# ssydasheng/GPflow-Slim

Hardware: AMD Instinct MI355X
Metric: GPR log-marginal-likelihood evals/sec + predict_f latency, fp64, N=32768 D=8 (higher is better)
Workload: dtype f64; 1 GPU; RBF(ARD) GPR log-marginal-likelihood, N=32768 D=8 R=1 fp64, X resident in HBM; n=32768, d=8, n_new=1024, parallelism=1 GPU (fused single-GPU path)

## Files before the change

gpflow-slim_amd/csrc/gps_handle.hip:

```cpp
#include "gps_ops.hpp"

extern "C" int gps_create(int device_id, gps_handle_t* out) {
  if (!out) return GPS_ERR_ARG;
  *out = nullptr;
  int count = 0;
  if (hipGetDeviceCount(&count) != hipSuccess || count <= 0) return GPS_ERR_HIP;
  if (device_id < 0 || device_id >= count) return GPS_ERR_ARG;
  gps_handle_t h = new gps_handle_s();
  h->device = device_id;
  if (hipSetDevice(device_id) != hipSuccess || hipGetDeviceProperties(&h->prop, device_id) != hipSuccess) {
    delete h;
    return GPS_ERR_HIP;
  }
  if (hipStreamCreateWithFlags(&h->stream, hipStreamNonBlocking) != hipSuccess) { delete h; return GPS_ERR_HIP; }
  for (int i = 0; i < 8; ++i) {
    if (hipEventCreate(&h->ev[i]) != hipSuccess) { delete h; return GPS_ERR_HIP; }
  }
  if (const char* v = getenv("GPS_GEMM_PAIR")) h->gemm_pair = atoi(v);
  if (const char* la = getenv("GPS_LOOKAHEAD")) h->potrf_lookahead = atoi(la);
  if (h->dInfo.ensure(64) != hipSuccess || h->dScal.ensure(4096) != hipSuccess) { delete h; return GPS_ERR_HIP; }
  *out = h;
  return GPS_OK;
}

// ... 187 lines not shown
  GPS_HIP(h, hipMemcpyAsync(h->dTmp2.p, B, bb, hipMemcpyHostToDevice, h->stream));
  GPS_HIP(h, hipMemcpyAsync(h->dTmp3.p, C, cb, hipMemcpyHostToDevice, h->stream));
  GemmBatch bt; bt.batch = batch; bt.a_rs = m; bt.b_rs = n; bt.c_rs = m;
  int rc = gps_launch_gemm_nt_ex(h, op, 0, tri, m, n, k, h->dTmp.d(), k, h->dTmp2.d(), k, h->dTmp3.d(), n, &bt);
  if (rc) return rc;
  GPS_HIP(h, hipMemcpyAsync(C, h->dTmp3.p, cb, hipMemcpyDeviceToHost, h->stream));
  GPS_HIP(h, hipStreamSynchronize(h->stream));
  return GPS_OK;
}

extern "C" int gps_diag_gemm_timeline(gps_handle_t h, int op, int lower, int64_t m, int64_t n, int64_t k, int reps,
                                      long long* stamps_out, int64_t cap_blocks, int64_t* nblocks, double* ms_per_launch) {
  if (!h || !stamps_out || cap_blocks <= 0 || reps <= 0) return GPS_ERR_ARG;
  GPS_HIP(h, hipSetDevice(h->device));
  return gps_run_gemm_timeline(h, op, lower, m, n, k, reps, stamps_out, cap_blocks, nblocks, ms_per_launch);
}

extern "C" int gps_diag_potrf_base_stamps(gps_handle_t h, int factor, double* us_out7) {
  if (!h || !us_out7) return GPS_ERR_ARG;
  GPS_HIP(h, hipSetDevice(h->device));
  const size_t bb = (size_t)GPS_TILE * GPS_TILE * 8;
  GPS_HIP(h, h->dTmp.ensure(4 * bb + 2048));
  std::vector<double> A((size_t)GPS_TILE * GPS_TILE, 0.0);
  for (int i = 0; i < GPS_TILE; ++i) for (int j = 0; j <= i; ++j) A[(size_t)i * GPS_TILE + j] = (i == j) ? 2.0 + 0.01 * i : 0.3 / (1.0 + i - j);
  double* dA = h->dTmp.d();
  long long* dS = (long long*)(dA + 3 * GPS_TILE * GPS_TILE);
  long long hs[96] = {0};
  const bool per_wave = getenv("GPS_PB_WAVE_STAMPS") != nullptr;
  for (int rep = 0; rep < 3; ++rep) {
    GPS_HIP(h, hipMemsetAsync(dS, 0, 96 * sizeof(long long), h->stream));
    if (per_wave) { const long long one = 1; GPS_HIP(h, hipMemcpyAsync(dS + 31, &one, sizeof(one), hipMemcpyHostToDevice, h->stream)); }
    GPS_HIP(h, hipMemcpyAsync(dA, A.data(), bb, hipMemcpyHostToDevice, h->stream));
    int rc = gps_launch_fill_info(h, (int*)h->dInfo.p, INT_MAX);
    if (rc) return rc;
    rc = gps_launch_potrf_base(h, dA, GPS_TILE, dA + GPS_TILE * GPS_TILE, getenv("GPS_PB_NO_T") ? nullptr : dA + 2 * GPS_TILE * GPS_TILE,
                               (int*)h->dInfo.p, 0, factor, dS);
    if (rc) return rc;
    GPS_HIP(h, hipMemcpyAsync(hs, dS, sizeof(hs), hipMemcpyDeviceToHost, h->stream));
    GPS_HIP(h, hipStreamSynchronize(h->stream));
  }
  for (int q = 0; q < 7; ++q) us_out7[q] = (double)(hs[q] - hs[0]) * 0.01;
  us_out7[0] = (double)(hs[8 + 2] - hs[8 + 1]) / ((double)(hs[2] - hs[1]) * 0.01);
  if (factor) {
    fprintf(stderr, "potrf_base phases (us): A (panel | update + inverse in its shadow) %.2f  B (next block column) %.2f\n", hs[16] * 0.01, hs[17] * 0.01);
    for (int g = 0; g < 8 && per_wave; ++g) {
      fprintf(stderr, "  step %d: per-wave end of phase A (us):", g);
      for (int w = 0; w < 8; ++w) fprintf(stderr, " %.2f", hs[32 + 8 * g + w] * 0.01);
      fprintf(stderr, "\n");
    }
  }
  return GPS_OK;
}

static int diag_trsm512_impl(gps_handle_t h, int64_t m, int backward, int panel, int reps, double* us_per_solve,
                             double* maxdiff_out, long long* stamps_out, int64_t cap_blocks) {
  if (!h || m <= 0 || m % GPS_TILE || reps <= 0 || !us_per_solve) return GPS_ERR_ARG;
  GPS_HIP(h, hipSetDevice(h->device));
  const i64 T = GPS_TILE, n = 4 * T;
  std::vector<double> L((size_t)n * n, 0.0), B((size_t)T * n);
  unsigned long long st = 88172645463325252ull;
  auto rnd = [&]() { st ^= st << 13; st ^= st >> 7; st ^= st << 17; return (double)(st >> 11) / 9007199254740992.0 - 0.5; };
  for (i64 i = 0; i < n; ++i) for (i64 j = 0; j <= i; ++j) L[i * n + j] = (i == j) ? 2.0 + 0.5 * (rnd() + 0.5) : 0.1 * rnd();
  for (auto& v : B) v = rnd();
  GPS_HIP(h, h->dTmp.ensure((size_t)2 * n * n * 8));
  GPS_HIP(h, h->dTmp3.ensure((size_t)8 * T * T * 8));
  GPS_HIP(h, h->dB.ensure((size_t)m * n * 8 * 3));
  double* dL = h->dTmp.d(); double* dU = dL + n * n; double* dInv = h->dTmp3.d(); double* dInvT = dInv + 4 * T * T;
  double* dBm = h->dB.d(); double* dB0 = dBm + m * n; double* dB1 = dB0 + m * n;
  GPS_HIP(h, hipMemcpyAsync(dL, L.data(), (size_t)n * n * 8, hipMemcpyHostToDevice, h->stream));
  for (i64 q = 0; q < m / T; ++q) GPS_HIP(h, hipMemcpyAsync(dB0 + q * T * n, B.data(), (size_t)T * n * 8, hipMemcpyHostToDevice, h->stream));
  int rc = gps_launch_transpose(h, dL, n, n, n, dU, n);
  if (rc) return rc;
  rc = gps_launch_fill_info(h, (int*)h->dInfo.p, INT_MAX);
  if (rc) return rc;
  HipOps ops{h, dInv, dInvT, (int*)h->dInfo.p};
  ops.factor = 0;
  for (i64 b = 0; b < 4 && !rc; ++b) rc = ops.potrf_base(dL + b * T * n + b * T, n, b, b * T);
  if (rc) return rc;
  Blocked<HipOps> bl(ops);
  const bool saved_ref = h->refine_now; const int saved_panel = h->trsm_panel;
  h->refine_now = false;
  auto solve = [&](double* X) -> int { return backward ? bl.trsm_rn_rec(dU, n, n, 0, X, n, m) : bl.trsm_rec(dL, n, n, 0, X, n, m); };
  hipEvent_t e0, e1;
  GPS_HIP(h, hipEventCreate(&e0)); GPS_HIP(h, hipEventCreate(&e1));
  float ms = 0.f;
  h->trsm_panel = panel;
  for (int pass = 0; pass < 2 && !rc; ++pass) {
    GPS_HIP(h, hipEventRecord(e0, h->stream));
    for (int it = 0; it < reps && !rc; ++it) {
      if (it == 0 || it == reps - 1) GPS_HIP(h, hipMemcpyAsync(dBm, dB0, (size_t)m * n * 8, hipMemcpyDeviceToDevice, h->stream));
      rc = solve(dBm);
    }
    GPS_HIP(h, hipEventRecord(e1, h->stream));
    GPS_HIP(h, hipStreamSynchronize(h->stream));
    GPS_HIP(h, hipEventElapsedTime(&ms, e0, e1));
  }
  if (!rc && stamps_out) {
    const i64 nb = std::min<i64>(m / 32, cap_blocks);
    GPS_HIP(h, h->dGemvWs.ensure((size_t)(m / 32) * 32 * sizeof(long long)));
    GPS_HIP(h, hipMemsetAsync(h->dGemvWs.p, 0, (size_t)(m / 32) * 32 * sizeof(long long), h->stream));
    GPS_HIP(h, hipMemcpyAsync(dBm, dB0, (size_t)m * n * 8, hipMemcpyDeviceToDevice, h->stream));
    h->tp_stamps = (long long*)h->dGemvWs.p;
    rc = solve(dBm);
    h->tp_stamps = nullptr;
    GPS_HIP(h, hipMemcpyAsync(stamps_out, h->dGemvWs.p, (size_t)nb * 32 * sizeof(long long), hipMemcpyDeviceToHost, h->stream));
    GPS_HIP(h, hipStreamSynchronize(h->stream));
// ... 102 lines not shown
```

gpflow-slim_amd/csrc/potrf_base.hip:

```cpp
#include "gps_common.hpp"

#define PB 128
#define PS 129
#define NT 512
typedef double v4d __attribute__((ext_vector_type(4)));
typedef double v2d_ __attribute__((ext_vector_type(2)));

#ifndef GPS_PB_WT
#define GPS_PB_WT 0
#endif
__device__ __forceinline__ void pb_store16(double* p, double2 v) {
#if GPS_PB_WT
  v2d_ w; w.x = v.x; w.y = v.y;
  asm volatile("global_store_dwordx4 %0, %1, off sc1\n\ts_nop 1" :: "v"(p), "v"(w) : "memory");
#else
  *reinterpret_cast<double2*>(p) = v;
#endif
}
typedef __attribute__((address_space(3))) int lds_int;

__device__ __forceinline__ void load_image(double* a, const double* __restrict__ A, i64 lda, int tid) {
  double2 v[16];
#pragma unroll
  for (int u = 0; u < 16; ++u) {
    const int idx = u * NT + tid;
    const int i = idx >> 6, j = (idx & 63) * 2;
    v[u] = *reinterpret_cast<const double2*>(A + (i64)i * lda + j);
  }
#pragma unroll
  for (int u = 0; u < 16; ++u) {
    const int idx = u * NT + tid;
    const int i = idx >> 6, j = (idx & 63) * 2;
    a[i * PS + j] = v[u].x;
    a[i * PS + j + 1] = v[u].y;
  }
}

__device__ __forceinline__ double x_elem(const double* a, const double* dinv, int r, int c) {
  double off = a[(r > c) ? (c * PS + r) : 0];
  double dia = dinv[r & (PB - 1)];
  asm volatile("" : "+v"(off), "+v"(dia));
  return (r > c) ? off : ((r == c) ? dia : 0.0);
}

#define PB_FMAC_DPP(d, a, b, k) asm volatile("v_fmac_f64_dpp %0, %1, -%2 row_newbcast:%3 row_mask:0xf bank_mask:0xf" : "+v"(d) : "v"(a), "v"(b), "n"(k))
#define PB_MOV_DPP(d, a, k) asm volatile("v_mov_b64_dpp %0, %1 row_newbcast:%2 row_mask:0xf bank_mask:0xf" : "=v"(d) : "v"(a), "n"(k))
#define PB_SCALE2(a, b, y) asm volatile("v_mul_f64 %0, %0, %2\n\tv_mul_f64 %1, %1, %2\n\ts_nop 1" : "+v"(a), "+v"(b) : "v"(y))
#define PB_UPD2(J, K) do { PB_FMAC_DPP(r[K], r[J], r[J], K); PB_FMAC_DPP(x[K], r[J], x[J], K); } while (0)

template <int J>
__device__ __forceinline__ void pb_pivot(double (&r)[16], double (&x)[16], double& p, double& y, double& sd, double& dd, int& bad) {
#define PB_FENCE() __builtin_amdgcn_sched_barrier(0)
  const double lj = sd * y;
  PB_SCALE2(r[J], x[J], y);
  PB_FENCE();
  const double pn = __builtin_fma(-lj, lj, dd);
  if constexpr (J + 1 < 16) PB_UPD2(J, J + 1);
// ... 111 lines not shown
  for (int rg = 0; rg < 4; ++rg) acc[rg] = pc[4 * rg * PS];
  for (int p = 0; p < np; ++p) {
    const int q = (p + 1 < np) ? p + 1 : p;
    double an[4], bn[4];
#pragma unroll
    for (int s4 = 0; s4 < 4; ++s4) { an[s4] = pa[16 * q + 4 * s4]; bn[s4] = pb[16 * q + 4 * s4]; }
    __builtin_amdgcn_sched_barrier(0);
#pragma unroll
    for (int s4 = 0; s4 < 4; ++s4) acc = __builtin_amdgcn_mfma_f64_16x16x4f64(-av[s4], bv[s4], acc, 0, 0, 0);
#pragma unroll
    for (int s4 = 0; s4 < 4; ++s4) { av[s4] = an[s4]; bv[s4] = bn[s4]; }
  }
#pragma unroll
  for (int rg = 0; rg < 4; ++rg) pc[4 * rg * PS] = acc[rg];
}

__device__ __forceinline__ int q_pull(int* counter, int lane) {
  int t = 0;
  if (lane == 0) t = atomicAdd(counter, 1);
  return __builtin_amdgcn_readfirstlane(t);
}

template <int NR>
__device__ __forceinline__ void store_L_rows(const double* a, double* __restrict__ A, i64 lda, int i0, int lane) {
  const int j = 2 * lane;
  char* base = reinterpret_cast<char*>(A + (i64)i0 * lda) + 16 * lane;
  const unsigned step = (unsigned)lda * 8u;
  double2 v[NR];
#pragma unroll
  for (int u = 0; u < NR; ++u) { v[u].x = a[(i0 + u) * PS + j]; v[u].y = a[(i0 + u) * PS + j + 1]; }
#pragma unroll
  for (int u = 0; u < NR; ++u) {
    const int i = i0 + u;
    v[u].x = (j <= i) ? v[u].x : 0.0;
    v[u].y = (j + 1 <= i) ? v[u].y : 0.0;
    pb_store16(reinterpret_cast<double*>(base + (size_t)(u * step)), v[u]);
  }
}
template <int NR>
__device__ __forceinline__ void store_inv_rows(const double* a, const double* dinv, double* __restrict__ Linv, int i0, int lane) {
  const int c = 2 * lane;
  double2 v[NR];
  double d[NR];
#pragma unroll
  for (int u = 0; u < NR; ++u) { v[u].x = a[c * PS + i0 + u]; v[u].y = a[(c + 1) * PS + i0 + u]; d[u] = dinv[i0 + u]; }
#pragma unroll
  for (int u = 0; u < NR; ++u) {
    const int i = i0 + u;
    v[u].x = (i > c) ? v[u].x : ((i == c) ? d[u] : 0.0);
    v[u].y = (i > c + 1) ? v[u].y : ((i == c + 1) ? d[u] : 0.0);
    pb_store16(Linv + i * PB + c, v[u]);
  }
}
__device__ __forceinline__ void inv_diag16(double* a, const double* dinv, int c) {
  const int rem = 15 - (c & 15);
  double x[16];
  x[0] = dinv[c];
#pragma unroll
  for (int d = 1; d < 16; ++d) {
    if (d <= rem) {
      const int i = c + d;
      double s = a[i * PS + c] * x[0];
#pragma unroll
      for (int t = 1; t < d; ++t) s += a[i * PS + c + t] * x[t];
      x[d] = -s * dinv[i];
    }
  }
#pragma unroll
  for (int d = 1; d < 16; ++d)
    if (d <= rem) a[c * PS + c + d] = x[d];
}

__device__ __forceinline__ void inv_row_tile(double* a, const double* dinv, int gp, int c, int fr, int fk) {
  v4d t0 = (v4d){0.0, 0.0, 0.0, 0.0}, t1 = (v4d){0.0, 0.0, 0.0, 0.0};
  const double* la = a + (16 * gp + fr) * PS + fk;
  const double* xb = a + (16 * c + fr) * PS + fk;
  double av[4], bv[4];
#pragma unroll
  for (int s = 0; s < 4; ++s) {
    av[s] = la[16 * c + 4 * s];
    bv[s] = x_elem(a, dinv, 16 * c + 4 * s + fk, 16 * c + fr);
  }
  for (int kb = c + 1; kb < gp; ++kb) {
    double an[4], bn[4];
#pragma unroll
    for (int s = 0; s < 4; ++s) { an[s] = la[16 * kb + 4 * s]; bn[s] = xb[16 * kb + 4 * s]; }
    t0 = __builtin_amdgcn_mfma_f64_16x16x4f64(av[0], bv[0], t0, 0, 0, 0);
    t1 = __builtin_amdgcn_mfma_f64_16x16x4f64(av[1], bv[1], t1, 0, 0, 0);
    t0 = __builtin_amdgcn_mfma_f64_16x16x4f64(av[2], bv[2], t0, 0, 0, 0);
    t1 = __builtin_amdgcn_mfma_f64_16x16x4f64(av[3], bv[3], t1, 0, 0, 0);
#pragma unroll
    for (int s = 0; s < 4; ++s) { av[s] = an[s]; bv[s] = bn[s]; }
  }
  double xv[4];
#pragma unroll
  for (int s = 0; s < 4; ++s) xv[s] = x_elem(a, dinv, 16 * gp + fr, 16 * gp + 4 * s + fk);
  t0 = __builtin_amdgcn_mfma_f64_16x16x4f64(av[0], bv[0], t0, 0, 0, 0);
  t1 = __builtin_amdgcn_mfma_f64_16x16x4f64(av[1], bv[1], t1, 0, 0, 0);
  t0 = __builtin_amdgcn_mfma_f64_16x16x4f64(av[2], bv[2], t0, 0, 0, 0);
  t1 = __builtin_amdgcn_mfma_f64_16x16x4f64(av[3], bv[3], t1, 0, 0, 0);
  t0 += t1;
  v4d z = (v4d){0.0, 0.0, 0.0, 0.0};
#pragma unroll
  for (int s = 0; s < 4; ++s) z = __builtin_amdgcn_mfma_f64_16x16x4f64(xv[s], t0[s], z, 0, 0, 0);
#pragma unroll
  for (int rg = 0; rg < 4; ++rg) a[(16 * c + fr) * PS + 16 * gp + fk + 4 * rg] = -z[rg];
}

__device__ __forceinline__ void potrf_base_body(char* smem_raw, double* __restrict__ A, i64 lda, double* __restrict__ Linv,
                                                double* __restrict__ LinvT, int* __restrict__ info, int row0, int factor,
                                                long long* __restrict__ stamps) {
#define STAMP(q) do { if (stamps && threadIdx.x == 0) { stamps[q] = (long long)wall_clock64(); stamps[8 + q] = (long long)clock64(); } } while (0)
  STAMP(0);
  double* a = reinterpret_cast<double*>(smem_raw);
  double* dinv = a + PB * PS;

  const int tid = threadIdx.x;
  const int lane = tid & 63, wave = __builtin_amdgcn_readfirstlane(tid >> 6);
  const int fr = lane & 15, fk = lane >> 4;

  int* q_mfma = reinterpret_cast<int*>(dinv + PB + 192);
  int* q_store = q_mfma + 9;
  lds_int* pflag = (lds_int*)(q_store + 8);
  __syncthreads();
  if (tid < 18) q_mfma[tid] = 0;
  load_image(a, A, lda, tid);
  __syncthreads();
  STAMP(1);

  int tail_row0 = 0;
  int flag_sum = 0;
  if (factor) {
    long long t_a = 0, t_b = 0, t0 = 0;
    for (int g = 0; g < 8; ++g) {
      const int o = 16 * g;
      const int nrows = PB - o - 16;
      const int npanel = nrows > 96 ? 3 : (nrows > 32 ? 2 : 1);
      if (stamps && (tid == 0 || (lane == 0 && stamps[31]))) t0 = (long long)wall_clock64();
      if (wave < npanel) {
        flag_sum += npanel - 1;
        panel_step_dpp(a, info, row0, o, lane, wave, npanel, pflag, flag_sum);
      } else if (g >= 1) {
        {
          const int n_inv = g - 1, n_ll = (g <= 6) ? 7 - g : 0, n_items = n_inv + n_ll;
          for (int it = q_pull(q_mfma + g, lane); it < n_items; it = q_pull(q_mfma + g, lane)) {
            if (n_inv > 0 && it == 0) inv_row_tile(a, dinv, g - 1, 0, fr, fk);
            else if (it - (n_inv > 0 ? 1 : 0) < n_ll) lookleft_tile(a, g + 1 + it - (n_inv > 0 ? 1 : 0), g + 1, g, fr, fk);
            else inv_row_tile(a, dinv, g - 1, it - n_ll, fr, fk);
          }
        }
        for (int it = q_pull(q_store + g, lane); it < 4; it = q_pull(q_store + g, lane))
          store_L_rows<4>(a, A, lda, 16 * (g - 1) + 4 * it, lane);
      }
      if (stamps && lane == 0 && stamps[31]) stamps[32 + 8 * g + wave] = (long long)wall_clock64() - t0;
      __syncthreads();
      if (stamps && tid == 0) { const long long t1 = (long long)wall_clock64(); t_a += t1 - t0; t0 = t1; }
      if (wave == 0) { }
      else {
        const int I = g + wave;
        if (I < 8) update_tile(a, I, g + 1, o, fr, fk);
      }
      __syncthreads();
      if (stamps && tid == 0) t_b += (long long)wall_clock64() - t0;
    }
    if (stamps && tid == 0) { stamps[16] = t_a; stamps[17] = t_b; stamps[18] = 0; }
    STAMP(2);
    STAMP(3);
    STAMP(4);
    if (wave < 7) inv_row_tile(a, dinv, 7, wave, fr, fk);
    {
      for (int it = q_pull(q_mfma + 8, lane); it < 4 + 28; it = q_pull(q_mfma + 8, lane)) {
        if (it < 4) store_L_rows<4>(a, A, lda, 112 + 4 * it, lane);
        else store_inv_rows<4>(a, dinv, Linv, 4 * (it - 4), lane);
      }
    }
    tail_row0 = 112;
    __syncthreads();
  } else {
    if (tid < PB) dinv[tid] = 1.0 / a[tid * PS + tid];
    __syncthreads();
    STAMP(2); STAMP(3);
    if (tid < PB) inv_diag16(a, dinv, tid);
    __syncthreads();
    STAMP(4);
    for (int gp = 1; gp < 8; ++gp) {
      if (wave < gp) inv_row_tile(a, dinv, gp, wave, fr, fk);
      __syncthreads();
    }
  }

  STAMP(5);
  {
    const int i0 = 0, w2 = PB / 2;
    for (int idx = tail_row0 * 64 + tid; idx < PB * PB / 2; idx += NT) {
      const int i = idx >> 6, c = (idx & 63) * 2;
      double2 v;
      v.x = x_elem(a, dinv, i, c);
      v.y = x_elem(a, dinv, i, c + 1);
      pb_store16(Linv + i * PB + c, v);
    }
    if (LinvT) {
      for (int idx = tid; idx < PB * w2; idx += NT) {
        const int c = idx / w2, i = i0 + 2 * (idx - c * w2);
        double2 v;
        v.x = x_elem(a, dinv, i, c);
        v.y = x_elem(a, dinv, i + 1, c);
        pb_store16(LinvT + c * PB + i, v);
      }
    }
  }
  __syncthreads();
  STAMP(6);
#undef STAMP
}


#define PB_LDS_BYTES ((PB * PS + PB + 192 + 10) * 8)

#ifndef GPS_PB_DEVICE_ONLY
__global__ __launch_bounds__(NT) __attribute__((amdgpu_waves_per_eu(2, 2))) void potrf_base_kernel(double* __restrict__ A, i64 lda,
                                                        double* __restrict__ Linv,
                                                        double* __restrict__ LinvT,
                                                        int* __restrict__ info, int row0,
                                                        int factor, long long* __restrict__ stamps) {
  extern __shared__ __attribute__((aligned(16))) char smem_raw[];
  potrf_base_body(smem_raw, A, lda, Linv, LinvT, info, row0, factor, stamps);
}

int gps_launch_potrf_base(gps_handle_t h, double* A, i64 lda, double* Linv_blk,
                          double* LinvT_blk, int* d_info, i64 row0, int factor, long long* d_stamps) {
  const size_t lds = (size_t)PB_LDS_BYTES;
  int rc0 = gps_dyn_lds(h, reinterpret_cast<const void*>(&potrf_base_kernel), (int)lds);
  if (rc0) return rc0;
  LaunchScope ls(h, KC_POTRF_BASE, 2.0 * PB * PB * PB / 3.0, 3.0 * PB * PB * 8.0);
  hipLaunchKernelGGL(potrf_base_kernel, dim3(1), dim3(NT), lds, h->stream, A, lda, Linv_blk,
                     LinvT_blk, d_info, (int)row0, factor, d_stamps);
  GPS_HIP(h, hipGetLastError());
  return GPS_OK;
}
#endif
```

gpflow-slim_amd/gpflowSlim/_backend.py:

```python
import ctypes
import os
import threading

import numpy as np

GPS_MAX_DIMS = 32
GPS_MAX_NODES = 64
GPS_MAX_STACK = 4

K_RBF, K_MATERN12, K_MATERN32, K_MATERN52, K_PERIODIC, K_WHITE, K_CONSTANT, K_EXPONENTIAL = 1, 2, 3, 4, 5, 6, 7, 8
K_SQDIST, K_EUCLID = 9, 10
K_ADD, K_MUL = 16, 17
K_NKN_LINROW, K_NKN_PRODUCT, K_NKN_ACT = 32, 33, 34

_c_double_p = ctypes.POINTER(ctypes.c_double)
_c_int_p = ctypes.POINTER(ctypes.c_int)
_i64 = ctypes.c_int64


class KernNode(ctypes.Structure):
    _fields_ = [("op", ctypes.c_int32),
                ("n_dims", ctypes.c_int32),
                ("active_dims", ctypes.c_int32 * GPS_MAX_DIMS),
                ("variance", ctypes.c_double),
# ... 93 lines not shown
                      _c_double_p, _c_double_p, _c_double_p, _c_int_p],
    "gps_fitc": [ctypes.c_void_p, ctypes.POINTER(KernNode), ctypes.c_int, _c_double_p, _i64, _c_double_p, _i64, _i64,
                 ctypes.c_double, ctypes.c_double, _c_double_p, _i64, _c_double_p, _i64, ctypes.c_int, _c_double_p,
                 _c_double_p, _c_double_p, _c_int_p],
    "gps_sparse_last_terms": [ctypes.c_void_p, _c_double_p],
    "gps_profile_enable": [ctypes.c_void_p, ctypes.c_int],
    "gps_profile_reset": [ctypes.c_void_p],
    "gps_profile_get": [ctypes.c_void_p, ctypes.c_char_p, ctypes.POINTER(_i64), _c_double_p, _c_double_p,
                        _c_double_p],
    "gps_last_stage_ms": [ctypes.c_void_p, _c_double_p],
    "gps_set_option": [ctypes.c_void_p, ctypes.c_char_p, ctypes.c_double],
    "gps_set_stream": [ctypes.c_void_p, ctypes.c_void_p, ctypes.c_int],
    "gps_dist_begin": [ctypes.c_void_p, ctypes.POINTER(KernNode), ctypes.c_int, ctypes.c_double, _c_double_p, _i64,
                       ctypes.c_int, ctypes.c_int, _i64, ctypes.POINTER(_i64), ctypes.POINTER(_i64)],
    "gps_dist_msg_doubles": [ctypes.c_void_p, _i64, ctypes.POINTER(_i64)],
    "gps_dist_set_comm": [ctypes.c_void_p, ctypes.c_void_p, ctypes.c_void_p],
    "gps_dist_set_comm_bufs": [ctypes.c_void_p, ctypes.POINTER(ctypes.c_void_p), ctypes.c_int],
    "gps_dist_comm_bufs_needed": [ctypes.c_void_p, _c_int_p],
    "gps_device_bytes": [ctypes.c_void_p, ctypes.POINTER(_i64)],
    "gps_dist_solve_begin": [ctypes.c_void_p, ctypes.POINTER(KernNode), ctypes.c_int, _c_double_p, _i64],
    "gps_dist_solve_pack": [ctypes.c_void_p, _i64, ctypes.c_int],
    "gps_dist_grad_begin": [ctypes.c_void_p],
    "gps_dist_grad_fwd_apply": [ctypes.c_void_p, _i64, ctypes.c_int],
    "gps_dist_grad_bwd_apply": [ctypes.c_void_p, _i64, ctypes.c_int],
    "gps_dist_grad_local": [ctypes.c_void_p, ctypes.POINTER(KernNode), ctypes.c_int, _c_double_p, ctypes.c_int, _c_int_p, _c_double_p],
    "gps_dist_grad_fold": [ctypes.c_void_p, ctypes.POINTER(KernNode), ctypes.c_int, _c_double_p, ctypes.c_int, _i64, _c_double_p,
                           ctypes.c_int, _c_int_p, _c_double_p],
    "gps_dist_lml_grad": [ctypes.c_void_p, ctypes.POINTER(KernNode), ctypes.c_int, ctypes.c_double, _c_double_p, _i64, _i64,
                          ctypes.c_int, ctypes.c_int, _c_double_p, _c_double_p, ctypes.c_int, _c_int_p, _c_double_p, _c_double_p,
                          _c_int_p],
    "gps_dist_solve_apply": [ctypes.c_void_p, _i64, ctypes.c_int],
    "gps_dist_solve_finish": [ctypes.c_void_p, ctypes.POINTER(KernNode), ctypes.c_int, _c_double_p, _c_double_p],
    "gps_dist_lml": [ctypes.c_void_p, ctypes.POINTER(KernNode), ctypes.c_int, ctypes.c_double, _c_double_p, _i64, _i64, ctypes.c_int,
                     ctypes.c_int, _c_double_p, _c_int_p],
    "gps_dist_predict": [ctypes.c_void_p, ctypes.POINTER(KernNode), ctypes.c_int, _c_double_p, _i64, ctypes.c_int, _c_double_p, _c_double_p],
    "gps_dist_panel_factor": [ctypes.c_void_p, _i64, ctypes.c_int],
    "gps_dist_unpack": [ctypes.c_void_p, _i64, ctypes.c_int],
    "gps_dist_update": [ctypes.c_void_p, _i64, _i64, _i64, ctypes.c_int],
    "gps_dist_set_bulk_stream": [ctypes.c_void_p, ctypes.c_void_p],
    "gps_dist_finish": [ctypes.c_void_p, _c_double_p, _c_int_p],
    "gps_comm_load": [ctypes.c_char_p],
    "gps_comm_version": [_c_int_p],
    "gps_comm_unique_id": [ctypes.c_void_p, ctypes.c_int],
    "gps_comm_init": [ctypes.c_void_p, ctypes.c_int, ctypes.c_int, ctypes.c_void_p, ctypes.c_int],
    "gps_comm_destroy": [ctypes.c_void_p],
    "gps_comm_abort": [ctypes.c_void_p],
    "gps_comm_exchange": [ctypes.c_void_p, ctypes.c_void_p, _i64, ctypes.c_int, ctypes.c_int, ctypes.c_int],
    "gps_comm_wait": [ctypes.c_void_p, ctypes.c_int],
    "gps_comm_allreduce": [ctypes.c_void_p, ctypes.c_void_p, _i64],
    "gps_comm_install_allreduce": [ctypes.c_void_p, ctypes.c_void_p, _i64],
    "gps_set_allreduce": [ctypes.c_void_p, ctypes.c_void_p, ctypes.c_void_p, ctypes.c_void_p, _i64],
    "gps_allreduce_doubles": [_i64, _i64, ctypes.POINTER(_i64)],
    "gps_diag_potrf_base_stamps": [ctypes.c_void_p, ctypes.c_int, _c_double_p],
    "gps_diag_mfma_f64": [ctypes.c_void_p, ctypes.c_int, _c_double_p, _c_int_p],
    "gps_diag_gemm_nt": [ctypes.c_void_p, ctypes.c_int, ctypes.c_int, _i64, _i64, _i64, _c_double_p, _c_double_p,
                         _c_double_p],
    "gps_diag_gemm_nt_batched": [ctypes.c_void_p, ctypes.c_int, ctypes.c_int, _i64, _i64, _i64, _i64, _c_double_p, _c_double_p,
                                 _c_double_p],
    "gps_diag_trsm512": [ctypes.c_void_p, _i64, ctypes.c_int, ctypes.c_int, ctypes.c_int, _c_double_p, _c_double_p],
    "gps_diag_trsm512_stamps": [ctypes.c_void_p, _i64, ctypes.c_int, ctypes.c_int, _c_double_p, ctypes.POINTER(ctypes.c_longlong), _i64],
    "gps_diag_trsm_leaf": [ctypes.c_void_p, _i64, ctypes.c_int, ctypes.c_int, ctypes.c_int, _c_double_p, _c_double_p],
    "gps_diag_set_cu_mask": [ctypes.c_void_p, ctypes.POINTER(ctypes.c_uint32), ctypes.c_int],
    "gps_diag_gemm_timeline": [ctypes.c_void_p, ctypes.c_int, ctypes.c_int, _i64, _i64, _i64, ctypes.c_int,
                               ctypes.POINTER(ctypes.c_longlong), _i64, ctypes.POINTER(ctypes.c_int64), _c_double_p],
}
EXPORTED_SYMBOLS = sorted(list(_SIGNATURES) + ["gps_last_error", "gps_comm_load_error"])
ALLREDUCE_FN = ctypes.CFUNCTYPE(ctypes.c_int, ctypes.c_void_p, ctypes.c_void_p, _i64)

_lib = None
_lib_lock = threading.Lock()


def _share_hip_runtime_with_torch():
    if os.environ.get("GPFLOWSLIM_NO_TORCH_RUNTIME"):
        return
    try:
        import importlib.util
        spec = importlib.util.find_spec("torch")
        if spec is None or not spec.submodule_search_locations:
            return
        cand = os.path.join(list(spec.submodule_search_locations)[0], "lib", "libamdhip64.so")
        if os.path.exists(cand):
            ctypes.CDLL(cand, mode=ctypes.RTLD_GLOBAL)
    except Exception:
        pass


def load_library():
    global _lib
    with _lib_lock:
        if _lib is not None:
            return _lib
        path = lib_path()
        if not os.path.exists(path):
            raise RuntimeError(
                "gpflowSlim (MI355X): HIP library not found at %s -- build it with "
                "`make -C gpflow-slim_amd/csrc` (or __graft_entry__.build()). There is no CPU fallback." % path)
        _share_hip_runtime_with_torch()
        lib = ctypes.CDLL(path)
        for name, argtypes in _SIGNATURES.items():
            try:
                fn = getattr(lib, name)
            except AttributeError:
                if os.environ.get("GPFLOWSLIM_HIP_LIB"):
                    continue
                raise
# ... 278 lines not shown
            raise NotPositiveDefiniteError(
                "Cholesky decomposition was not successful: leading minor of order %d is not positive definite" % info.value)
        return lml.value

    def dist_predict(self, prog, Xnew, r, exchange_mode):
        Xnew = _f64(Xnew)
        n_new = Xnew.shape[0]
        mean = np.empty((n_new, max(r, 1)))
        var = np.empty(n_new)
        self._check(self._lib.gps_dist_predict(self._h, prog, len(prog), _ptr(Xnew) if n_new else None, n_new, int(exchange_mode),
                                               _ptr(mean) if n_new else None, _ptr(var) if n_new else None), "gps_dist_predict")
        return mean[:, :r], var

    def dist_panel_factor(self, j, buf):
        self._check(self._lib.gps_dist_panel_factor(self._h, int(j), int(buf)), "gps_dist_panel_factor")

    def dist_unpack(self, j, buf):
        self._check(self._lib.gps_dist_unpack(self._h, int(j), int(buf)), "gps_dist_unpack")

    def dist_update(self, j, c_lo, c_hi, lane=0):
        self._check(self._lib.gps_dist_update(self._h, int(j), int(c_lo), int(c_hi), int(lane)), "gps_dist_update")

    def dist_set_bulk_stream(self, hip_stream):
        self._check(self._lib.gps_dist_set_bulk_stream(self._h, ctypes.c_void_p(hip_stream) if hip_stream else None),
                    "gps_dist_set_bulk_stream")

    def dist_finish(self):
        lml = ctypes.c_double(0)
        info = ctypes.c_int(0)
        self._check(self._lib.gps_dist_finish(self._h, ctypes.byref(lml), ctypes.byref(info)), "gps_dist_finish")
        if info.value > 0:
            raise NotPositiveDefiniteError(
                "Cholesky decomposition was not successful: leading minor of order %d is not positive definite"
                % info.value)
        return lml.value

    def diag_mfma_f64(self, waves_per_simd=1):
        tf = ctypes.c_double(0)
        ok = ctypes.c_int(0)
        self._check(self._lib.gps_diag_mfma_f64(self._h, waves_per_simd, ctypes.byref(tf), ctypes.byref(ok)),
                    "gps_diag_mfma_f64")
        return tf.value, bool(ok.value)

    def diag_gemm_nt(self, op, lower, A, B, C):
        A, B = _f64(A), _f64(B)
        C = np.array(C, dtype=np.float64, order="C", copy=True)
        m, k = A.shape
        n = B.shape[0]
        assert B.shape[1] == k and C.shape == (m, n)
        self._check(self._lib.gps_diag_gemm_nt(self._h, op, int(lower), m, n, k, _ptr(A), _ptr(B), _ptr(C)),
                    "gps_diag_gemm_nt")
        return C

    def diag_gemm_nt_batched(self, op, tri, A, B, C):
        A, B = _f64(A), _f64(B)
        C = np.array(C, dtype=np.float64, order="C", copy=True)
        batch, m, k = A.shape
        n = B.shape[1]
        assert B.shape == (batch, n, k) and C.shape == (batch, m, n)
        self._check(self._lib.gps_diag_gemm_nt_batched(self._h, op, int(tri), batch, m, n, k, _ptr(A), _ptr(B), _ptr(C)),
                    "gps_diag_gemm_nt_batched")
        return C

    def diag_trsm_leaf(self, m, mode, upper=False, reps=50):
        us, res = ctypes.c_double(0), ctypes.c_double(0)
        self._check(self._lib.gps_diag_trsm_leaf(self._h, int(m), int(mode), int(bool(upper)), int(reps),
                                                 ctypes.byref(us), ctypes.byref(res)), "gps_diag_trsm_leaf")
        return us.value, res.value

    def diag_trsm512(self, m, backward=False, panel=True, reps=20):
        us, diff = ctypes.c_double(0), ctypes.c_double(0)
        self._check(self._lib.gps_diag_trsm512(self._h, int(m), int(bool(backward)), int(bool(panel)), int(reps),
                                               ctypes.byref(us), ctypes.byref(diff)), "gps_diag_trsm512")
        return us.value, diff.value

    def diag_trsm512_stamps(self, m, backward=False, reps=5):
        nb = int(m) // 32
        buf = np.zeros((nb, 32), dtype=np.int64)
        us = ctypes.c_double(0)
        self._check(self._lib.gps_diag_trsm512_stamps(self._h, int(m), int(bool(backward)), int(reps), ctypes.byref(us),
                                                      buf.ctypes.data_as(ctypes.POINTER(ctypes.c_longlong)), nb), "gps_diag_trsm512_stamps")
        return us.value, buf

    def diag_set_cu_mask(self, words):
        arr = (ctypes.c_uint32 * len(words))(*[int(w) & 0xffffffff for w in words])
        self._check(self._lib.gps_diag_set_cu_mask(self._h, arr, len(words)), "gps_diag_set_cu_mask")

    def diag_gemm_timeline(self, op, lower, m, n, k, reps=5, cap_blocks=1 << 17):
        st = np.zeros((cap_blocks, 6), dtype=np.int64)
        nb, ms = ctypes.c_int64(), ctypes.c_double()
        self._check(self._lib.gps_diag_gemm_timeline(self._h, op, int(lower), m, n, k, reps,
                                                     st.ctypes.data_as(ctypes.POINTER(ctypes.c_longlong)), cap_blocks,
                                                     ctypes.byref(nb), ctypes.byref(ms)), "gps_diag_gemm_timeline")
        return ms.value, st[:nb.value]

    def kmat(self, prog, X, X2=None, diag_add=0.0):
        X = _f64(X)
        n, d = X.shape
        if X2 is None:
            out = np.empty((n, n))
            self._check(self._lib.gps_kmat(self._h, prog, len(prog), _ptr(X), n, None, 0, d, float(diag_add),
                                           _ptr(out)), "gps_kmat")
        else:
            X2 = _f64(X2)
            if X2.shape[1] != d:
                raise ValueError("X and X2 must have the same number of columns")
# ... 477 lines not shown
```

include/gpflowslim_hip.h:

```cpp
#ifndef GPFLOWSLIM_HIP_H
#define GPFLOWSLIM_HIP_H

#include <stdint.h>

#ifdef __cplusplus
extern "C" {
#endif

#define GPS_MAX_DIMS   32
#define GPS_MAX_NODES  64
#define GPS_MAX_STACK   4

#define GPS_OK              0
#define GPS_ERR_ARG        -1
#define GPS_ERR_HIP        -2
#define GPS_ERR_STATE      -3
#define GPS_ERR_UNSUPPORTED -4

enum gps_kern_op {
  GPS_K_RBF      = 1,
  GPS_K_MATERN12 = 2,
  GPS_K_MATERN32 = 3,
  GPS_K_MATERN52 = 4,
  GPS_K_PERIODIC = 5,
// ... 163 lines not shown

int gps_profile_enable(gps_handle_t h, int on);
int gps_profile_reset(gps_handle_t h);
int gps_profile_get(gps_handle_t h, const char* klass, int64_t* launches,
                    double* ms, double* flops, double* bytes);
int gps_last_stage_ms(gps_handle_t h, double* out5);

int gps_set_stream(gps_handle_t h, void* hip_stream, int external);
int gps_dist_begin(gps_handle_t h, const gps_kern_node_t* prog, int n_nodes, double noise_var,
                   const double* resid, int64_t r, int nparts, int part, int64_t nb,
                   int64_t* n_panels, int64_t* msg_doubles_max);
int gps_dist_msg_doubles(gps_handle_t h, int64_t j, int64_t* out);
int gps_dist_set_comm(gps_handle_t h, void* dev_buf0, void* dev_buf1);
int gps_dist_set_comm_bufs(gps_handle_t h, void* const* dev_bufs, int count);
int gps_dist_comm_bufs_needed(gps_handle_t h, int* count);
int gps_dist_lml(gps_handle_t h, const gps_kern_node_t* prog, int n_nodes, double noise_var, const double* resid,
                 int64_t r, int64_t nb, int lookahead, int exchange_mode, double* lml, int* info);
int gps_dist_solve_begin(gps_handle_t h, const gps_kern_node_t* prog, int n_nodes, const double* Xnew, int64_t n_new);
int gps_dist_solve_pack(gps_handle_t h, int64_t j, int buf);
int gps_dist_solve_apply(gps_handle_t h, int64_t j, int buf);
int gps_dist_solve_finish(gps_handle_t h, const gps_kern_node_t* prog, int n_nodes, double* mean_out, double* var_out);
int gps_dist_predict(gps_handle_t h, const gps_kern_node_t* prog, int n_nodes, const double* Xnew, int64_t n_new,
                     int exchange_mode, double* mean_out, double* var_out);
int gps_dist_grad_begin(gps_handle_t h);
int gps_dist_grad_fwd_apply(gps_handle_t h, int64_t j, int buf);
int gps_dist_grad_bwd_apply(gps_handle_t h, int64_t j, int buf);
int gps_dist_grad_local(gps_handle_t h, const gps_kern_node_t* prog, int n_nodes, double* sums_out, int cap,
                        int* n_slots_out, double* kinv_resid_out);
int gps_dist_grad_fold(gps_handle_t h, const gps_kern_node_t* prog, int n_nodes, const double* rank_sums, int P,
                       int64_t stride, double* grad_slots, int n_slots_cap, int* n_slots_out, double* grad_noise);
int gps_dist_lml_grad(gps_handle_t h, const gps_kern_node_t* prog, int n_nodes, double noise_var, const double* resid,
                      int64_t r, int64_t nb, int lookahead, int exchange_mode, double* lml, double* grad_slots,
                      int n_slots_cap, int* n_slots_out, double* grad_noise, double* kinv_resid, int* info);
int gps_device_bytes(gps_handle_t h, int64_t* bytes);
int gps_dist_set_bulk_stream(gps_handle_t h, void* hip_stream);
int gps_dist_panel_factor(gps_handle_t h, int64_t j, int buf);
int gps_dist_unpack(gps_handle_t h, int64_t j, int buf);
int gps_dist_update(gps_handle_t h, int64_t j, int64_t c_lo, int64_t c_hi, int lane);
int gps_dist_finish(gps_handle_t h, double* lml, int* info);

int gps_set_option(gps_handle_t h, const char* key, double value);

int gps_diag_mfma_f64(gps_handle_t h, int waves_per_simd, double* tflops,
                      int* layout_ok);
int gps_diag_gemm_nt(gps_handle_t h, int op, int lower, int64_t m, int64_t n,
                     int64_t k, const double* A, const double* B, double* C);
int gps_diag_gemm_nt_batched(gps_handle_t h, int op, int tri, int64_t batch, int64_t m, int64_t n, int64_t k,
                             const double* A, const double* B, double* C);
int gps_diag_gemm_timeline(gps_handle_t h, int op, int lower, int64_t m, int64_t n, int64_t k, int reps,
                           long long* stamps_out, int64_t cap_blocks, int64_t* nblocks,
                           double* ms_per_launch);
int gps_diag_set_cu_mask(gps_handle_t h, const uint32_t* mask, int n_words);
int gps_diag_potrf_base_stamps(gps_handle_t h, int factor, double* out7);

int gps_diag_trsm512(gps_handle_t h, int64_t m, int backward, int panel, int reps, double* us_per_solve,
                     double* maxdiff_out);
int gps_diag_trsm512_stamps(gps_handle_t h, int64_t m, int backward, int reps, double* us_per_solve, long long* stamps_out,
                            int64_t cap_blocks);
int gps_diag_trsm_leaf(gps_handle_t h, int64_t m, int mode, int upper, int reps, double* us_per_launch,
                       double* resid_out);

#ifdef __cplusplus
}
#endif
#endif
```

Measured before the change: 5.536 evals/s.

## Overlap last-block inverse with final panel step in potrf base kernel

In the 128x128 diagonal-block Cholesky kernel, idle waves at step 7 now start the last-row inverse partial sums and the leftover L-row stores while the panel waves run. Only the final MFMA multiply remains after the panel completes. The transposed-inverse stores for the tail are folded into the shared work queue, and the generic tail loop is limited to the remaining rows. This shortens the serial tail of each diagonal factorization but adds register pressure and more complex wave-role logic. Two optional variants sit behind compile flags that default off, and a diagnostic entry point is added to test a single block.

```diff
diff --git a/gpflow-slim_amd/csrc/gps_handle.hip b/gpflow-slim_amd/csrc/gps_handle.hip
--- a/gpflow-slim_amd/csrc/gps_handle.hip
+++ b/gpflow-slim_amd/csrc/gps_handle.hip
@@ -263,6 +263,30 @@
   return GPS_OK;
 }
 
+extern "C" int gps_diag_potrf_base_block(gps_handle_t h, const double* A, int factor, int with_T, double* L_out, double* Linv_out,
+                                         double* LinvT_out, int* info) {
+  if (!h || !A || !L_out || !Linv_out || (with_T && !LinvT_out)) return GPS_ERR_ARG;
+  GPS_HIP(h, hipSetDevice(h->device));
+  const size_t bb = (size_t)GPS_TILE * GPS_TILE * 8;
+  GPS_HIP(h, h->dTmp.ensure(4 * bb + 2048));
+  double* dA = h->dTmp.d();
+  GPS_HIP(h, hipMemcpyAsync(dA, A, bb, hipMemcpyHostToDevice, h->stream));
+  GPS_HIP(h, hipMemsetAsync(dA + GPS_TILE * GPS_TILE, 0xff, 2 * bb, h->stream));
+  int rc = gps_launch_fill_info(h, (int*)h->dInfo.p, INT_MAX);
+  if (rc) return rc;
+  rc = gps_launch_potrf_base(h, dA, GPS_TILE, dA + GPS_TILE * GPS_TILE, with_T ? dA + 2 * GPS_TILE * GPS_TILE : nullptr,
+                             (int*)h->dInfo.p, 0, factor, nullptr);
+  if (rc) return rc;
+  GPS_HIP(h, hipMemcpyAsync(L_out, dA, bb, hipMemcpyDeviceToHost, h->stream));
+  GPS_HIP(h, hipMemcpyAsync(Linv_out, dA + GPS_TILE * GPS_TILE, bb, hipMemcpyDeviceToHost, h->stream));
+  if (with_T) GPS_HIP(h, hipMemcpyAsync(LinvT_out, dA + 2 * GPS_TILE * GPS_TILE, bb, hipMemcpyDeviceToHost, h->stream));
+  int hinfo = 0;
+  GPS_HIP(h, hipMemcpyAsync(&hinfo, h->dInfo.p, sizeof(int), hipMemcpyDeviceToHost, h->stream));
+  GPS_HIP(h, hipStreamSynchronize(h->stream));
+  if (info) *info = (hinfo == INT_MAX) ? 0 : hinfo;
+  return GPS_OK;
+}
+
 static int diag_trsm512_impl(gps_handle_t h, int64_t m, int backward, int panel, int reps, double* us_per_solve,
                              double* maxdiff_out, long long* stamps_out, int64_t cap_blocks) {
   if (!h || m <= 0 || m % GPS_TILE || reps <= 0 || !us_per_solve) return GPS_ERR_ARG;
diff --git a/gpflow-slim_amd/csrc/potrf_base.hip b/gpflow-slim_amd/csrc/potrf_base.hip
--- a/gpflow-slim_amd/csrc/potrf_base.hip
+++ b/gpflow-slim_amd/csrc/potrf_base.hip
@@ -3,6 +3,12 @@
 #define PB 128
 #define PS 129
 #define NT 512
+#ifndef PB_EARLY7
+#define PB_EARLY7 0
+#endif
+#ifndef PB_PARTNER_VALU
+#define PB_PARTNER_VALU 0
+#endif
 typedef double v4d __attribute__((ext_vector_type(4)));
 typedef double v2d_ __attribute__((ext_vector_type(2)));
 
@@ -220,6 +226,21 @@
     pb_store16(Linv + i * PB + c, v[u]);
   }
 }
+template <int NR>
+__device__ __forceinline__ void store_invT_rows(const double* a, const double* dinv, double* __restrict__ LinvT, int c0, int ncol, int lane) {
+  const int i = 2 * lane;
+  double2 v[NR];
+  double d[NR];
+#pragma unroll
+  for (int u = 0; u < NR; ++u) { v[u].x = a[(c0 + u) * PS + i]; v[u].y = a[(c0 + u) * PS + i + 1]; d[u] = dinv[c0 + u]; }
+#pragma unroll
+  for (int u = 0; u < NR; ++u) {
+    const int c = c0 + u;
+    v[u].x = (i > c) ? v[u].x : ((i == c) ? d[u] : 0.0);
+    v[u].y = (i + 1 > c) ? v[u].y : ((i + 1 == c) ? d[u] : 0.0);
+    if (i < ncol) pb_store16(LinvT + c * PB + i, v[u]);
+  }
+}
 __device__ __forceinline__ void inv_diag16(double* a, const double* dinv, int c) {
   const int rem = 15 - (c & 15);
   double x[16];
@@ -239,7 +260,12 @@
     if (d <= rem) a[c * PS + c + d] = x[d];
 }
 
-__device__ __forceinline__ void inv_row_tile(double* a, const double* dinv, int gp, int c, int fr, int fk) {
+__device__ __forceinline__ void inv_row_xdiag(const double* a, const double* dinv, int gp, int fr, int fk, double (&xv)[4]) {
+#pragma unroll
+  for (int s = 0; s < 4; ++s) xv[s] = x_elem(a, dinv, 16 * gp + fr, 16 * gp + 4 * s + fk);
+}
+__device__ __forceinline__ v4d inv_row_sum(const double* a, const double* dinv, int gp, int c, int fr, int fk, bool reg_last, v4d xlast,
+                                           bool with_xv, double (&xv)[4]) {
   v4d t0 = (v4d){0.0, 0.0, 0.0, 0.0}, t1 = (v4d){0.0, 0.0, 0.0, 0.0};
   const double* la = a + (16 * gp + fr) * PS + fk;
   const double* xb = a + (16 * c + fr) * PS + fk;
@@ -249,7 +275,8 @@
     av[s] = la[16 * c + 4 * s];
     bv[s] = x_elem(a, dinv, 16 * c + 4 * s + fk, 16 * c + fr);
   }
-  for (int kb = c + 1; kb < gp; ++kb) {
+  const int kend = reg_last ? gp - 1 : gp;
+  for (int kb = c + 1; kb < kend; ++kb) {
     double an[4], bn[4];
 #pragma unroll
     for (int s = 0; s < 4; ++s) { an[s] = la[16 * kb + 4 * s]; bn[s] = xb[16 * kb + 4 * s]; }
@@ -260,19 +287,38 @@
 #pragma unroll
     for (int s = 0; s < 4; ++s) { av[s] = an[s]; bv[s] = bn[s]; }
   }
-  double xv[4];
-#pragma unroll
-  for (int s = 0; s < 4; ++s) xv[s] = x_elem(a, dinv, 16 * gp + fr, 16 * gp + 4 * s + fk);
+  if (reg_last) {
+    double an[4];
+#pragma unroll
+    for (int s = 0; s < 4; ++s) an[s] = la[16 * (gp - 1) + 4 * s];
+    t0 = __builtin_amdgcn_mfma_f64_16x16x4f64(av[0], bv[0], t0, 0, 0, 0);
+    t1 = __builtin_amdgcn_mfma_f64_16x16x4f64(av[1], bv[1], t1, 0, 0, 0);
+    t0 = __builtin_amdgcn_mfma_f64_16x16x4f64(av[2], bv[2], t0, 0, 0, 0);
+    t1 = __builtin_amdgcn_mfma_f64_16x16x4f64(av[3], bv[3], t1, 0, 0, 0);
+#pragma unroll
+    for (int s = 0; s < 4; ++s) { av[s] = an[s]; bv[s] = xlast[s]; }
+  }
+  if (with_xv) inv_row_xdiag(a, dinv, gp, fr, fk, xv);
   t0 = __builtin_amdgcn_mfma_f64_16x16x4f64(av[0], bv[0], t0, 0, 0, 0);
   t1 = __builtin_amdgcn_mfma_f64_16x16x4f64(av[1], bv[1], t1, 0, 0, 0);
   t0 = __builtin_amdgcn_mfma_f64_16x16x4f64(av[2], bv[2], t0, 0, 0, 0);
   t1 = __builtin_amdgcn_mfma_f64_16x16x4f64(av[3], bv[3], t1, 0, 0, 0);
   t0 += t1;
+  return t0;
+}
+__device__ __forceinline__ v4d inv_row_finish(double* a, int gp, int c, int fr, int fk, v4d t0, const double (&xv)[4]) {
   v4d z = (v4d){0.0, 0.0, 0.0, 0.0};
 #pragma unroll
   for (int s = 0; s < 4; ++s) z = __builtin_amdgcn_mfma_f64_16x16x4f64(xv[s], t0[s], z, 0, 0, 0);
-#pragma unroll
-  for (int rg = 0; rg < 4; ++rg) a[(16 * c + fr) * PS + 16 * gp + fk + 4 * rg] = -z[rg];
+  z = -z;
+#pragma unroll
+  for (int rg = 0; rg < 4; ++rg) a[(16 * c + fr) * PS + 16 * gp + fk + 4 * rg] = z[rg];
+  return z;
+}
+__device__ __forceinline__ v4d inv_row_tile(double* a, const double* dinv, int gp, int c, int fr, int fk) {
+  double xv[4];
+  const v4d t = inv_row_sum(a, dinv, gp, c, fr, fk, false, (v4d){0.0, 0.0, 0.0, 0.0}, true, xv);
+  return inv_row_finish(a, gp, c, fr, fk, t, xv);
 }
 
 __device__ __forceinline__ void potrf_base_body(char* smem_raw, double* __restrict__ A, i64 lda, double* __restrict__ Linv,
@@ -290,8 +336,10 @@
   int* q_mfma = reinterpret_cast<int*>(dinv + PB + 192);
   int* q_store = q_mfma + 9;
   lds_int* pflag = (lds_int*)(q_store + 8);
+  [[maybe_unused]] lds_int* done7 = pflag + 1;
+  [[maybe_unused]] int* q_early = q_mfma + 7;
   __syncthreads();
-  if (tid < 18) q_mfma[tid] = 0;
+  if (tid < 20) q_mfma[tid] = 0;
   load_image(a, A, lda, tid);
   __syncthreads();
   STAMP(1);
@@ -300,6 +348,8 @@
   int flag_sum = 0;
   if (factor) {
     long long t_a = 0, t_b = 0, t0 = 0;
+    const int c7 = (wave == 4) ? 6 : (wave < 4 ? wave - 1 : 10 - wave);
+    v4d t7 = (v4d){0.0, 0.0, 0.0, 0.0};
     for (int g = 0; g < 8; ++g) {
       const int o = 16 * g;
       const int nrows = PB - o - 16;
@@ -308,9 +358,29 @@
       if (wave < npanel) {
         flag_sum += npanel - 1;
         panel_step_dpp(a, info, row0, o, lane, wave, npanel, pflag, flag_sum);
+#if PB_EARLY7
+        if (g == 7 && lane == 0) __hip_atomic_store(done7, 1, __ATOMIC_RELAXED, __HIP_MEMORY_SCOPE_WORKGROUP);
+#endif
+      } else if (g == 7) {
+        double xv[4];
+        v4d x6 = (v4d){0.0, 0.0, 0.0, 0.0};
+        if (c7 < 6) x6 = inv_row_tile(a, dinv, 6, c7, fr, fk);
+        t7 = inv_row_sum(a, dinv, 7, c7, fr, fk, c7 < 6, x6, false, xv);
+        for (int it = q_pull(q_store + g, lane); it < 4; it = q_pull(q_store + g, lane))
+          store_L_rows<4>(a, A, lda, 16 * (g - 1) + 4 * it, lane);
+#if PB_EARLY7
+        while (!__hip_atomic_load(done7, __ATOMIC_RELAXED, __HIP_MEMORY_SCOPE_WORKGROUP)) {
+          const int it = q_pull(q_early, lane);
+          if (it >= 24) break;
+          store_inv_rows<4>(a, dinv, Linv, 4 * it, lane);
+        }
+#endif
       } else if (g >= 1) {
+#if PB_PARTNER_VALU
+        if (!(wave >= 4 && wave - 4 < npanel))
+#endif
         {
-          const int n_inv = g - 1, n_ll = (g <= 6) ? 7 - g : 0, n_items = n_inv + n_ll;
+          const int n_inv = g - 1, n_ll = 7 - g, n_items = n_inv + n_ll;
           for (int it = q_pull(q_mfma + g, lane); it < n_items; it = q_pull(q_mfma + g, lane)) {
             if (n_inv > 0 && it == 0) inv_row_tile(a, dinv, g - 1, 0, fr, fk);
             else if (it - (n_inv > 0 ? 1 : 0) < n_ll) lookleft_tile(a, g + 1 + it - (n_inv > 0 ? 1 : 0), g + 1, g, fr, fk);
@@ -335,11 +405,22 @@
     STAMP(2);
     STAMP(3);
     STAMP(4);
-    if (wave < 7) inv_row_tile(a, dinv, 7, wave, fr, fk);
+    if (wave >= 1) {
+      double xv[4];
+      inv_row_xdiag(a, dinv, 7, fr, fk, xv);
+      inv_row_finish(a, 7, c7, fr, fk, t7, xv);
+    }
     {
-      for (int it = q_pull(q_mfma + 8, lane); it < 4 + 28; it = q_pull(q_mfma + 8, lane)) {
+      int e0 = 0;
+#if PB_EARLY7
+      e0 = __builtin_amdgcn_readfirstlane(*q_early);
+      e0 = e0 < 24 ? e0 : 24;
+#endif
+      const int n_inv = 28 - e0, n_items = 4 + n_inv + (LinvT ? 32 : 0);
+      for (int it = q_pull(q_mfma + 8, lane); it < n_items; it = q_pull(q_mfma + 8, lane)) {
         if (it < 4) store_L_rows<4>(a, A, lda, 112 + 4 * it, lane);
-        else store_inv_rows<4>(a, dinv, Linv, 4 * (it - 4), lane);
+        else if (it < 4 + n_inv) store_inv_rows<4>(a, dinv, Linv, 4 * (e0 + it - 4), lane);
+        else store_invT_rows<4>(a, dinv, LinvT, 4 * (it - 4 - n_inv), 112, lane);
       }
     }
     tail_row0 = 112;
@@ -359,7 +440,7 @@
 
   STAMP(5);
   {
-    const int i0 = 0, w2 = PB / 2;
+    const int i0 = tail_row0, sh = tail_row0 ? 3 : 6, w2 = 1 << sh;
     for (int idx = tail_row0 * 64 + tid; idx < PB * PB / 2; idx += NT) {
       const int i = idx >> 6, c = (idx & 63) * 2;
       double2 v;
@@ -369,7 +450,7 @@
     }
     if (LinvT) {
       for (int idx = tid; idx < PB * w2; idx += NT) {
-        const int c = idx / w2, i = i0 + 2 * (idx - c * w2);
+        const int c = idx >> sh, i = i0 + 2 * (idx - c * w2);
         double2 v;
         v.x = x_elem(a, dinv, i, c);
         v.y = x_elem(a, dinv, i + 1, c);
diff --git a/gpflow-slim_amd/gpflowSlim/_backend.py b/gpflow-slim_amd/gpflowSlim/_backend.py
--- a/gpflow-slim_amd/gpflowSlim/_backend.py
+++ b/gpflow-slim_amd/gpflowSlim/_backend.py
@@ -169,6 +169,8 @@
     "gps_set_allreduce": [ctypes.c_void_p, ctypes.c_void_p, ctypes.c_void_p, ctypes.c_void_p, _i64],
     "gps_allreduce_doubles": [_i64, _i64, ctypes.POINTER(_i64)],
     "gps_diag_potrf_base_stamps": [ctypes.c_void_p, ctypes.c_int, _c_double_p],
+    "gps_diag_potrf_base_block": [ctypes.c_void_p, _c_double_p, ctypes.c_int, ctypes.c_int, _c_double_p, _c_double_p, _c_double_p,
+                                  _c_int_p],
     "gps_diag_mfma_f64": [ctypes.c_void_p, ctypes.c_int, _c_double_p, _c_int_p],
     "gps_diag_gemm_nt": [ctypes.c_void_p, ctypes.c_int, ctypes.c_int, _i64, _i64, _i64, _c_double_p, _c_double_p,
                          _c_double_p],
@@ -553,6 +555,15 @@
                     "gps_diag_gemm_nt")
         return C
 
+    def diag_potrf_base_block(self, A, factor=True, with_T=True):
+        A = _f64(A)
+        assert A.shape == (128, 128)
+        L, Li, LiT = np.empty_like(A), np.empty_like(A), np.empty_like(A)
+        info = ctypes.c_int(0)
+        self._check(self._lib.gps_diag_potrf_base_block(self._h, _ptr(A), int(bool(factor)), int(bool(with_T)), _ptr(L), _ptr(Li),
+                                                        _ptr(LiT), ctypes.byref(info)), "gps_diag_potrf_base_block")
+        return L, Li, (LiT if with_T else None), info.value
+
     def diag_gemm_nt_batched(self, op, tri, A, B, C):
         A, B = _f64(A), _f64(B)
         C = np.array(C, dtype=np.float64, order="C", copy=True)
diff --git a/include/gpflowslim_hip.h b/include/gpflowslim_hip.h
--- a/include/gpflowslim_hip.h
+++ b/include/gpflowslim_hip.h
@@ -239,6 +239,8 @@
                            double* ms_per_launch);
 int gps_diag_set_cu_mask(gps_handle_t h, const uint32_t* mask, int n_words);
 int gps_diag_potrf_base_stamps(gps_handle_t h, int factor, double* out7);
+int gps_diag_potrf_base_block(gps_handle_t h, const double* A, int factor, int with_T, double* L_out, double* Linv_out,
+                              double* LinvT_out, int* info);
 
 int gps_diag_trsm512(gps_handle_t h, int64_t m, int backward, int panel, int reps, double* us_per_solve,
                      double* maxdiff_out);
```

After: 5.536 evals/s, median of 3. Within noise of the previous version (-0.0%).
